# TUMFTM/CamRaDepth

Hardware: AMD Instinct MI355X
Metric: training images/sec at 256x416 bf16 (higher is better)
Workload: dtype bf16; 1 GPU; CamRaDepth base (image+radar) train step, 8x7x256x416 per GPU, bf16 MFMA / fp32 accumulate, diffGradNorm + OneCycleLR, Dropout2d/DropPath on; global_batch=8, parallelism=dp1, hip_graph=True

## Files before the change

### camradepth_amd/csrc/wgrad3x3.hip

```cpp
#include <stdlib.h>
#include "common.h"

namespace {

struct Wg3K {
  const bf16_t* x; int x_ld; int Cin;
  const bf16_t* dy; int dy_ld; int Cout;
  int B, H, W;
  int strips_x;
  int rows_per_wg;
  int S, nchunks;
  long long total_rows;
  long long x_bytes, dy_bytes;
  crd_sum_t* dw; crd_sum_t* dbias;
  float* dw_part;
};

constexpr int XS = 6, YS = 4;
constexpr int XPX = 40;
constexpr int XLD = 64;
typedef __attribute__((address_space(3))) void* lds_ptr;
__device__ __forceinline__ int swz128(int r) { return (r & 3) ^ ((r >> 3) & 1); }
__device__ __forceinline__ int swz256(int r) { return (r & 3) | (((r >> 3) & 1) << 2); }
__device__ __forceinline__ int swz192(int r) { return (r >> 3) & 1; }
template <int COT>
__device__ __forceinline__ int swz_y(int r) { return COT == 128 ? swz256(r) : (COT == 96 ? swz192(r) : (COT == 64 ? swz128(r) : 0)); }

__device__ __forceinline__ s16x4 tr_read3(const bf16_t* p) {
  return __builtin_amdgcn_ds_read_tr16_b64_v4i16((__attribute__((address_space(3))) s16x4*)(p));
}

template <int WCO, int WCI, int TCO, int RPS>
__global__ __launch_bounds__(512) void k_wgrad3x3(Wg3K a) {
  constexpr int XSr = XS * RPS, YSr = YS * RPS;
  static_assert(WCO * WCI == 8, "8 waves");
  constexpr int NT = 4 / WCI;
  constexpr int COT = WCO * TCO * 16;
  constexpr int YGRP = 32 * COT * 2 / 1024;
  extern __shared__ __attribute__((aligned(16))) bf16_t lds[];
  bf16_t* sX = lds;
  bf16_t* sY = lds + XSr * XPX * XLD;

  const int t = threadIdx.x, l = t & 63;
  const int wv = __builtin_amdgcn_readfirstlane(t >> 6);
  const int wco = wv / WCI, wci = wv % WCI;
  const int chunk = (int)blockIdx.x / a.S, split = (int)blockIdx.x - chunk * a.S;
  const int c0 = chunk * XLD;
  const unsigned OOB = 0x80000000u;

  f32x4 acc[9][TCO][NT];
#pragma unroll
  for (int tp = 0; tp < 9; ++tp)
#pragma unroll
    for (int i = 0; i < TCO; ++i)
#pragma unroll
      for (int j = 0; j < NT; ++j) acc[tp][i][j] = f32x4{0.f, 0.f, 0.f, 0.f};
  const int q = l >> 4, prow = (l & 15) >> 2, pcol = (l & 3) * 4;
  int yoff[TCO][2], xoff[3][NT][2];
#pragma unroll
  for (int i = 0; i < TCO; ++i)
#pragma unroll
    for (int h = 0; h < 2; ++h) {
      const int r = 8 * q + prow + 4 * h;
      yoff[i][h] = r * COT + (((wco * TCO + i) ^ swz_y<COT>(r)) << 4) + pcol;
    }
#pragma unroll
  for (int kx = 0; kx < 3; ++kx)
#pragma unroll
    for (int j = 0; j < NT; ++j)
#pragma unroll
      for (int h = 0; h < 2; ++h) {
        const int r = 8 * q + prow + kx + 4 * h;
        xoff[kx][j][h] = r * XLD + (((wci * NT + j) ^ swz128(r)) << 4) + pcol;
      }
  const bool do_bias = a.dbias != nullptr && chunk == 0 && t < a.Cout;
  float bsum = 0.f;

  long long sr = (long long)split * a.rows_per_wg;
  long long sr_end = sr + a.rows_per_wg;
  if (sr_end > a.total_rows) sr_end = a.total_rows;

  const int xpix = 8 * wv + (l >> 3);
  const int xgr = l & 7;
  const int ylin = 64 * wv + l;
  const int ypix = ylin / (COT / 8);
  const int ygr = ylin % (COT / 8);

  while (sr < sr_end) {
    const long long strip = sr / a.H;
    const int y0 = (int)(sr - strip * a.H);
    long long seg_end = (strip + 1) * a.H;
    if (seg_end > sr_end) seg_end = sr_end;
    const int y1 = y0 + (int)(seg_end - sr);
    const int b = __builtin_amdgcn_readfirstlane((int)(strip / a.strips_x));
    const int sx = (int)(strip - (long long)b * a.strips_x);
    const int x0 = sx * 32;
    const crd_rsrc_t rx = make_rsrc(a.x + (long long)b * a.H * a.W * a.x_ld, (unsigned)a.x_bytes);
    const crd_rsrc_t ry = make_rsrc(a.dy + (long long)b * a.H * a.W * a.dy_ld, (unsigned)a.dy_bytes);

    auto issue_x = [&](int h) {
#if defined(__HIP_DEVICE_COMPILE__)
      if (wv < 5) {
        const int ix = x0 - 1 + xpix, ch = c0 + ((((xgr >> 1) ^ swz128(xpix)) << 1) | (xgr & 1)) * 8;
        const bool ok = (unsigned)h < (unsigned)a.H && (unsigned)ix < (unsigned)a.W && xpix < 34 && ch < a.Cin;
        const unsigned off = ok ? (unsigned)((((long long)h * a.W + ix) * a.x_ld + ch) * 2) : OOB;
        lds_dma16(rx, (unsigned)(uintptr_t)(lds_ptr)(sX + (((h + 1) % XSr) * XPX + 8 * wv) * XLD), off);
      }
#else
      (void)h;
#endif
    };
    auto issue_y = [&](int r) {
#if defined(__HIP_DEVICE_COMPILE__)
      if (wv < YGRP) {
        const int ix = x0 + ypix, co = ((((ygr >> 1) ^ swz_y<COT>(ypix)) << 1) | (ygr & 1)) * 8;
        const bool ok = r < y1 && ix < a.W && co < a.Cout;
        const unsigned off = ok ? (unsigned)((((long long)r * a.W + ix) * a.dy_ld + co) * 2) : OOB;
        lds_dma16(ry, (unsigned)(uintptr_t)(lds_ptr)(sY + (r % YSr) * 32 * COT + 512 * wv), off);
      }
#else
      (void)r;
#endif
    };

    asm volatile("s_waitcnt vmcnt(0) lgkmcnt(0)\n\ts_barrier" ::: "memory");
    issue_x(y0 - 1);
    issue_x(y0);
#pragma unroll
    for (int s = 0; s < 3; ++s)
#pragma unroll
      for (int r = 0; r < RPS; ++r) { issue_y(y0 + s * RPS + r); issue_x(y0 + s * RPS + 1 + r); }

    for (int y = y0; y < y1; y += RPS) {
      if (wv < 5 && wv < YGRP) wait_vm<4 * RPS>();
      else if (wv < 5 || wv < YGRP) wait_vm<2 * RPS>();
      asm volatile("s_waitcnt lgkmcnt(0)\n\ts_barrier" ::: "memory");
#pragma unroll
      for (int r = 0; r < RPS; ++r) { issue_y(y + 3 * RPS + r); issue_x(y + 3 * RPS + 1 + r); }

      const bool mfma_on = c0 + wci * NT * 16 < a.Cin;
      if (!mfma_on && !do_bias) continue;
#pragma unroll
      for (int rr = 0; rr < RPS; ++rr) {
        const int yy = y + rr;
        if (rr > 0 && yy >= y1) break;
        const bf16_t* yrow = sY + (yy % YSr) * 32 * COT;
        if (mfma_on) {
        bf16x8 af[TCO];
#pragma unroll
        for (int i = 0; i < TCO; ++i) {
          s16x4 lo = tr_read3(yrow + yoff[i][0]), hi = tr_read3(yrow + yoff[i][1]);
          union { bf16x8 v; s16x4 h[2]; } u;
          u.h[0] = lo; u.h[1] = hi;
          af[i] = u.v;
        }
#pragma unroll
        for (int ky = 0; ky < 3; ++ky) {
          const bf16_t* xrow = sX + ((yy + ky) % XSr) * XPX * XLD;
#pragma unroll
          for (int kx = 0; kx < 3; ++kx) {
#pragma unroll
            for (int j = 0; j < NT; ++j) {
              s16x4 lo = tr_read3(xrow + xoff[kx][j][0]), hi = tr_read3(xrow + xoff[kx][j][1]);
              union { bf16x8 v; s16x4 h[2]; } u;
              u.h[0] = lo; u.h[1] = hi;
#pragma unroll
              for (int i = 0; i < TCO; ++i)
                acc[ky * 3 + kx][i][j] = __builtin_amdgcn_mfma_f32_16x16x32_bf16(af[i], u.v, acc[ky * 3 + kx][i][j], 0, 0, 0);
            }
          }
        }
        }
        if (do_bias) {
#pragma unroll 8
          for (int r = 0; r < 32; ++r) bsum += bf2f(yrow[r * COT + ((((t >> 4) ^ swz_y<COT>(r)) << 4) | (t & 15))]);
        }
      }
    }
    sr = seg_end;
  }

  const int Ktot = 9 * a.Cin;
#pragma unroll
  for (int tp = 0; tp < 9; ++tp)
#pragma unroll
    for (int i = 0; i < TCO; ++i)
#pragma unroll
      for (int j = 0; j < NT; ++j) {
        const int ci = c0 + (wci * NT + j) * 16 + (l & 15);
#pragma unroll
        for (int r = 0; r < 4; ++r) {
          const int co = (wco * TCO + i) * 16 + (l >> 4) * 4 + r;
          if (co < a.Cout && ci < a.Cin) {
            const long long off = (long long)co * Ktot + tp * a.Cin + ci;
            if (a.dw_part) a.dw_part[(long long)split * a.Cout * Ktot + off] = acc[tp][i][j][r];
            else grad_add(a.dw + off, acc[tp][i][j][r]);
          }
        }
      }
  if (do_bias) grad_add(a.dbias + t, bsum);
}

int plan_rows(long long total_rows, int Cin, int& rows_per_wg, int budget, int cap) {
  const int chunks = cdiv(Cin, XLD);
  const int W = budget > 0 ? budget : 256;
  long long S = W / chunks;
  if (S < 1) S = 1;
  if (cap > 0 && S > cap) S = cap;
  if (S > total_rows / 8) S = total_rows / 8 > 0 ? total_rows / 8 : 1;
  rows_per_wg = (int)((total_rows + S - 1) / S);
  return (int)((total_rows + rows_per_wg - 1) / rows_per_wg);
}

template <int WCO, int WCI, int TCO, int RPS>
Wg3K prepare_w3r(const Wg3K& k0, int budget, int partial_capacity, size_t& lds) {
  Wg3K k = k0;
  constexpr int COT = WCO * TCO * 16;
  lds = (size_t)RPS * (XS * XPX * XLD + YS * 32 * COT) * sizeof(bf16_t);
  k.nchunks = cdiv(k.Cin, XLD);
  k.S = plan_rows(k.total_rows, k.Cin, k.rows_per_wg, budget, k.dw_part ? partial_capacity : 0);
  return k;
}

template <int WCO, int WCI, int TCO, int RPS>
int launch_w3r(const Wg3K& k0, hipStream_t st, int budget, int partial_capacity, char* label, int capacity) {
  size_t lds;
  const Wg3K k = prepare_w3r<WCO, WCI, TCO, RPS>(k0, budget, partial_capacity, lds);
  if (label) {
    const int n = snprintf(label, capacity, "k_wgrad3x3<%d,%d,%d,%d>/S=%d,rows_per_wg=%d,chunks=%d", WCO, WCI, TCO, RPS, k.S, k.rows_per_wg, k.nchunks);
    CRD_CHECK_ARG(n < capacity, "crd_conv_wgrad_route: the label needs %d bytes, capacity is %d", n + 1, capacity);
    return CRD_OK;
  }
  crd_reserve_lds_once<&k_wgrad3x3<WCO, WCI, TCO, RPS>>((int)lds, "k_wgrad3x3");
  hipLaunchKernelGGL((k_wgrad3x3<WCO, WCI, TCO, RPS>), dim3(k.nchunks * k.S), dim3(512), lds, st, k);
  CRD_LAUNCH_CHECK("crd_conv_wgrad(3x3 streaming)");
  return CRD_OK;
}

template <int WCO, int WCI, int TCO>
int launch_w3(const Wg3K& k, hipStream_t st, int budget, int partial_capacity, char* label, int capacity) {
  static int rps = -1;
  if (rps < 0) rps = crd_dev_int("CRD_W3_RPS", 2);
  return rps == 1 ? launch_w3r<WCO, WCI, TCO, 1>(k, st, budget, partial_capacity, label, capacity)
                  : launch_w3r<WCO, WCI, TCO, 2>(k, st, budget, partial_capacity, label, capacity);
}

int w3_dispatch(const crd_wgrad_desc* d, hipStream_t st, char* label, int capacity) {
  Wg3K k;
  k.x = reinterpret_cast<const bf16_t*>(d->x) + d->x_coff; k.x_ld = d->x_ld; k.Cin = d->Cin;
  k.dy = reinterpret_cast<const bf16_t*>(d->dy) + d->dy_coff; k.dy_ld = d->dy_ld; k.Cout = d->Cout;
  k.B = d->B; k.H = d->IH; k.W = d->IW;
  k.strips_x = cdiv(d->IW, 32);
  k.total_rows = (long long)d->B * k.strips_x * d->IH;
  k.rows_per_wg = 0;
  k.x_bytes = (long long)d->IH * d->IW * d->x_ld * 2;
  k.dy_bytes = (long long)d->IH * d->IW * d->dy_ld * 2;
  CRD_UNSUPPORTED(k.x_bytes < (1ll << 31) && k.dy_bytes < (1ll << 31), "crd_conv_wgrad: image too large for 32-bit byte offsets");
  k.dw = d->dw; k.dbias = d->dbias;
  k.dw_part = d->dw_partials;
  CRD_CHECK_ARG(d->dw_partials == nullptr || d->dw_partial_capacity >= 1, "crd_conv_wgrad: dw_partials needs a capacity >= 1");
  CRD_CHECK_ARG(d->wg_budget >= 0, "crd_conv_wgrad: wg_budget must be >= 0");
  CRD_UNSUPPORTED(d->Cout <= 128, "crd_conv_wgrad: the streaming 3x3 kernel covers at most 128 output channels");
  if (d->Cout <= 32) return launch_w3<2, 4, 1>(k, st, d->wg_budget, d->dw_partial_capacity, label, capacity);
  if (d->Cout <= 64) return launch_w3<2, 4, 2>(k, st, d->wg_budget, d->dw_partial_capacity, label, capacity);
  if (d->Cout <= 96) return launch_w3<2, 4, 3>(k, st, d->wg_budget, d->dw_partial_capacity, label, capacity);
  if (crd_dev_int("CRD_W3_T22", 0)) return launch_w3<4, 2, 2>(k, st, d->wg_budget, d->dw_partial_capacity, label, capacity);
  return launch_w3<2, 4, 4>(k, st, d->wg_budget, d->dw_partial_capacity, label, capacity);
}

}

int crd_wgrad3x3_stream(const crd_wgrad_desc* d, hipStream_t st) { return w3_dispatch(d, st, nullptr, 0); }
int crd_wgrad3x3_route(const crd_wgrad_desc* d, char* label, int capacity) { return w3_dispatch(d, nullptr, label, capacity); }

int crd_wgrad3x3_splits(const crd_wgrad_desc* d) {
  int rows = 0;
  return plan_rows((long long)d->B * cdiv(d->IW, 32) * d->IH, d->Cin, rows, d->wg_budget, d->dw_partial_capacity > 0 ? d->dw_partial_capacity : 0);
}
```

Baseline: 473.8 images/s.

## Software-pipeline LDS fragment reads against MFMA in 3x3 weight-grad kernel

Restructures the wgrad3x3 main loop so LDS transposed reads for the next tap or row are issued while MFMAs for the current tap run, double-buffering x fragments and prefetching the next row's first fragments across the barrier. The dy ring gains one more stage (YS 4 to 5) so dy loads run a row further ahead. Per-lane address pieces are hoisted out of the DMA issue lambdas, and global requests are staggered across waves. The aim is to hide LDS latency and cut issue overhead, at the cost of more registers and LDS, which may lower occupancy or cause spills.

Result: no change. 477.8 images/s (median of 6 runs) (+0.8%).

```diff
diff --git a/camradepth_amd/csrc/wgrad3x3.hip b/camradepth_amd/csrc/wgrad3x3.hip
--- a/camradepth_amd/csrc/wgrad3x3.hip
+++ b/camradepth_amd/csrc/wgrad3x3.hip
@@ -1,4 +1,5 @@
 #include <stdlib.h>
+#include <type_traits>
 #include "common.h"
 
 namespace {
@@ -16,7 +17,7 @@
   float* dw_part;
 };
 
-constexpr int XS = 6, YS = 4;
+constexpr int XS = 6, YS = 5;
 constexpr int XPX = 40;
 constexpr int XLD = 64;
 typedef __attribute__((address_space(3))) void* lds_ptr;
@@ -34,12 +35,14 @@
 __global__ __launch_bounds__(512) void k_wgrad3x3(Wg3K a) {
   constexpr int XSr = XS * RPS, YSr = YS * RPS;
   static_assert(WCO * WCI == 8, "8 waves");
+  static_assert(RPS == 1 || RPS == 2, "the odd-length tail below is written for at most two rows per step");
   constexpr int NT = 4 / WCI;
   constexpr int COT = WCO * TCO * 16;
   constexpr int YGRP = 32 * COT * 2 / 1024;
   extern __shared__ __attribute__((aligned(16))) bf16_t lds[];
   bf16_t* sX = lds;
   bf16_t* sY = lds + XSr * XPX * XLD;
+  const unsigned ldsX = (unsigned)(uintptr_t)(lds_ptr)sX, ldsY = ldsX + XSr * XPX * XLD * 2;
 
   const int t = threadIdx.x, l = t & 63;
   const int wv = __builtin_amdgcn_readfirstlane(t >> 6);
@@ -98,13 +101,18 @@
     const crd_rsrc_t rx = make_rsrc(a.x + (long long)b * a.H * a.W * a.x_ld, (unsigned)a.x_bytes);
     const crd_rsrc_t ry = make_rsrc(a.dy + (long long)b * a.H * a.W * a.dy_ld, (unsigned)a.dy_bytes);
 
+    const int xrow_bytes = a.W * a.x_ld * 2, yrow_bytes = a.W * a.dy_ld * 2;
+    const int xix = x0 - 1 + xpix, xch = c0 + ((((xgr >> 1) ^ swz128(xpix)) << 1) | (xgr & 1)) * 8;
+    const bool xlane_ok = (unsigned)xix < (unsigned)a.W && xpix < 34 && xch < a.Cin;
+    const int xlane_off = (xix * a.x_ld + xch) * 2;
+    const int yix = x0 + ypix, yco = ((((ygr >> 1) ^ swz_y<COT>(ypix)) << 1) | (ygr & 1)) * 8;
+    const bool ylane_ok = yix < a.W && yco < a.Cout;
+    const int ylane_off = (yix * a.dy_ld + yco) * 2;
     auto issue_x = [&](int h) {
 #if defined(__HIP_DEVICE_COMPILE__)
       if (wv < 5) {
-        const int ix = x0 - 1 + xpix, ch = c0 + ((((xgr >> 1) ^ swz128(xpix)) << 1) | (xgr & 1)) * 8;
-        const bool ok = (unsigned)h < (unsigned)a.H && (unsigned)ix < (unsigned)a.W && xpix < 34 && ch < a.Cin;
-        const unsigned off = ok ? (unsigned)((((long long)h * a.W + ix) * a.x_ld + ch) * 2) : OOB;
-        lds_dma16(rx, (unsigned)(uintptr_t)(lds_ptr)(sX + (((h + 1) % XSr) * XPX + 8 * wv) * XLD), off);
+        const unsigned off = (xlane_ok && (unsigned)h < (unsigned)a.H) ? (unsigned)(h * xrow_bytes + xlane_off) : OOB;
+        lds_dma16(rx, ldsX + (unsigned)((((h + 1) % XSr) * XPX + 8 * wv) * XLD * 2), off);
       }
 #else
       (void)h;
@@ -113,68 +121,117 @@
     auto issue_y = [&](int r) {
 #if defined(__HIP_DEVICE_COMPILE__)
       if (wv < YGRP) {
-        const int ix = x0 + ypix, co = ((((ygr >> 1) ^ swz_y<COT>(ypix)) << 1) | (ygr & 1)) * 8;
-        const bool ok = r < y1 && ix < a.W && co < a.Cout;
-        const unsigned off = ok ? (unsigned)((((long long)r * a.W + ix) * a.dy_ld + co) * 2) : OOB;
-        lds_dma16(ry, (unsigned)(uintptr_t)(lds_ptr)(sY + (r % YSr) * 32 * COT + 512 * wv), off);
+        const unsigned off = (ylane_ok && r < y1) ? (unsigned)(r * yrow_bytes + ylane_off) : OOB;
+        lds_dma16(ry, ldsY + (unsigned)(((r % YSr) * 32 * COT + 512 * wv) * 2), off);
       }
 #else
       (void)r;
 #endif
     };
 
+    auto rendezvous = [&]() {
+      if (wv < 5 && wv < YGRP) wait_vm<4 * RPS>();
+      else if (wv < 5 || wv < YGRP) wait_vm<2 * RPS>();
+      asm volatile("s_waitcnt lgkmcnt(0)\n\ts_barrier" ::: "memory");
+    };
+    auto read_y = [&](int yy, bf16x8 (&af)[TCO]) {
+      const bf16_t* yrow = sY + (yy % YSr) * 32 * COT;
+#pragma unroll
+      for (int i = 0; i < TCO; ++i) {
+        union { bf16x8 v; s16x4 h[2]; } u;
+        u.h[0] = tr_read3(yrow + yoff[i][0]); u.h[1] = tr_read3(yrow + yoff[i][1]);
+        af[i] = u.v;
+      }
+    };
+    auto read_x = [&](int yy, int ky, bf16x8 (&xf)[3][NT]) {
+      const bf16_t* xrow = sX + ((yy + ky) % XSr) * XPX * XLD;
+#pragma unroll
+      for (int kx = 0; kx < 3; ++kx)
+#pragma unroll
+        for (int j = 0; j < NT; ++j) {
+          union { bf16x8 v; s16x4 h[2]; } u;
+          u.h[0] = tr_read3(xrow + xoff[kx][j][0]); u.h[1] = tr_read3(xrow + xoff[kx][j][1]);
+          xf[kx][j] = u.v;
+        }
+    };
+    auto taps = [&](int ky, const bf16x8 (&af)[TCO], const bf16x8 (&xf)[3][NT]) {
+#pragma unroll
+      for (int kx = 0; kx < 3; ++kx)
+#pragma unroll
+        for (int j = 0; j < NT; ++j)
+#pragma unroll
+          for (int i = 0; i < TCO; ++i)
+            acc[ky * 3 + kx][i][j] = __builtin_amdgcn_mfma_f32_16x16x32_bf16(af[i], xf[kx][j], acc[ky * 3 + kx][i][j], 0, 0, 0);
+    };
+    auto bias_row = [&](int yy) {
+      const bf16_t* yrow = sY + (yy % YSr) * 32 * COT;
+#pragma unroll 8
+      for (int r = 0; r < 32; ++r) bsum += bf2f(yrow[r * COT + ((((t >> 4) ^ swz_y<COT>(r)) << 4) | (t & 15))]);
+    };
+    const bool mfma_on = c0 + wci * NT * 16 < a.Cin;
+
     asm volatile("s_waitcnt vmcnt(0) lgkmcnt(0)\n\ts_barrier" ::: "memory");
     issue_x(y0 - 1);
     issue_x(y0);
 #pragma unroll
+    for (int r = 0; r < RPS; ++r) issue_y(y0 + r);
+#pragma unroll
     for (int s = 0; s < 3; ++s)
 #pragma unroll
-      for (int r = 0; r < RPS; ++r) { issue_y(y0 + s * RPS + r); issue_x(y0 + s * RPS + 1 + r); }
-
-    for (int y = y0; y < y1; y += RPS) {
-      if (wv < 5 && wv < YGRP) wait_vm<4 * RPS>();
-      else if (wv < 5 || wv < YGRP) wait_vm<2 * RPS>();
-      asm volatile("s_waitcnt lgkmcnt(0)\n\ts_barrier" ::: "memory");
-#pragma unroll
-      for (int r = 0; r < RPS; ++r) { issue_y(y + 3 * RPS + r); issue_x(y + 3 * RPS + 1 + r); }
-
-      const bool mfma_on = c0 + wci * NT * 16 < a.Cin;
-      if (!mfma_on && !do_bias) continue;
-#pragma unroll
-      for (int rr = 0; rr < RPS; ++rr) {
-        const int yy = y + rr;
-        if (rr > 0 && yy >= y1) break;
-        const bf16_t* yrow = sY + (yy % YSr) * 32 * COT;
-        if (mfma_on) {
-        bf16x8 af[TCO];
-#pragma unroll
-        for (int i = 0; i < TCO; ++i) {
-          s16x4 lo = tr_read3(yrow + yoff[i][0]), hi = tr_read3(yrow + yoff[i][1]);
-          union { bf16x8 v; s16x4 h[2]; } u;
-          u.h[0] = lo; u.h[1] = hi;
-          af[i] = u.v;
+      for (int r = 0; r < RPS; ++r) { issue_y(y0 + (s + 1) * RPS + r); issue_x(y0 + s * RPS + 1 + r); }
+    rendezvous();
+    bf16x8 caf[TCO], cx0[3][NT];
+    if (mfma_on) { read_y(y0, caf); read_x(y0, 0, cx0); }
+
+    auto requests = [&](int y) {
+#pragma unroll
+      for (int r = 0; r < RPS; ++r) { issue_y(y + 4 * RPS + r); issue_x(y + 3 * RPS + 1 + r); }
+    };
+    auto rows = [&](auto rows_c, auto head_c, int y) {
+      constexpr int K = 3 * decltype(rows_c)::value;
+      constexpr bool HEAD = decltype(head_c)::value, DB = NT == 1;
+      bf16x8 af[TCO], xb[2][3][NT], naf[TCO], nx0[3][NT];
+#pragma unroll
+      for (int k = 0; k < K; ++k) {
+        const int kn = DB ? k + 1 : k;
+        if (kn >= 1 && kn < K) {
+          if (kn == 3) read_y(y + 1, af);
+          read_x(y + kn / 3, kn % 3, xb[DB ? (kn & 1) : 0]);
         }
-#pragma unroll
-        for (int ky = 0; ky < 3; ++ky) {
-          const bf16_t* xrow = sX + ((yy + ky) % XSr) * XPX * XLD;
-#pragma unroll
-          for (int kx = 0; kx < 3; ++kx) {
-#pragma unroll
-            for (int j = 0; j < NT; ++j) {
-              s16x4 lo = tr_read3(xrow + xoff[kx][j][0]), hi = tr_read3(xrow + xoff[kx][j][1]);
-              union { bf16x8 v; s16x4 h[2]; } u;
-              u.h[0] = lo; u.h[1] = hi;
-#pragma unroll
-              for (int i = 0; i < TCO; ++i)
-                acc[ky * 3 + kx][i][j] = __builtin_amdgcn_mfma_f32_16x16x32_bf16(af[i], u.v, acc[ky * 3 + kx][i][j], 0, 0, 0);
-            }
-          }
-        }
-        }
-        if (do_bias) {
-#pragma unroll 8
-          for (int r = 0; r < 32; ++r) bsum += bf2f(yrow[r * COT + ((((t >> 4) ^ swz_y<COT>(r)) << 4) | (t & 15))]);
-        }
+        if (HEAD && k == K - 1) { read_y(y + K / 3, naf); read_x(y + K / 3, 0, nx0); }
+        if (k == 0) taps(0, caf, cx0);
+        else if (k < 3) taps(k, caf, xb[DB ? (k & 1) : 0]);
+        else taps(k - 3, af, xb[DB ? (k & 1) : 0]);
+        __builtin_amdgcn_sched_group_barrier(0x100, 64, 0);
+        __builtin_amdgcn_sched_group_barrier(0x008, 64, 0);
+        __builtin_amdgcn_sched_barrier(0);
+        if (HEAD && k == 0 && wv < 4) requests(y);
+        if (HEAD && k == K / 2 && wv >= 4) requests(y);
+      }
+      if (HEAD) {
+#pragma unroll
+        for (int i = 0; i < TCO; ++i) caf[i] = naf[i];
+#pragma unroll
+        for (int kx = 0; kx < 3; ++kx)
+#pragma unroll
+          for (int j = 0; j < NT; ++j) cx0[kx][j] = nx0[kx][j];
+      }
+    };
+
+    int y = y0;
+    for (; y + RPS <= y1; y += RPS) {
+      if (mfma_on) rows(std::integral_constant<int, RPS>{}, std::true_type{}, y);
+      else requests(y);
+      if (do_bias) {
+#pragma unroll
+        for (int r = 0; r < RPS; ++r) bias_row(y + r);
+      }
+      rendezvous();
+    }
+    if constexpr (RPS == 2) {
+      if (y < y1) {
+        if (mfma_on) rows(std::integral_constant<int, 1>{}, std::false_type{}, y);
+        if (do_bias) bias_row(y);
       }
     }
     sr = seg_end;
```
